# rhoposit/self-attention-tacotron

Hardware: AMD Instinct MI355X
Metric: teacher-forced mel frames/sec, LJSpeech batch=32, 1/2/4/8 MI355X (higher is better)
Workload: dtype fp32; 1 GPU; LJSpeech self-attention-tacotron.json teacher-forced training step (fwd + BPTT + Adam), configs[1]; global_batch=32, per_gpu_batch=32, chars=200, mel_frames=1000, num_mels=80, r=2, decoder_steps=500, parallelism=dp1, hip_graph=True, params=6227928

## Files before the change

self-attention-tacotron_amd/csrc/decoder_persistent.hip:

```cpp
#include "sat_common.h"
#include "persistent.h"

namespace sat {
namespace {

constexpr int kG = 8;
constexpr int kGW = 32;
constexpr int kPN = 32;
constexpr int kUBmax = 4;
constexpr int kU = 256, kM1 = 256, kM2 = 32, kD1 = 224, kD2 = 32, kF = 5, kKW = 10;
constexpr int kK0 = kM1 + kM2 + kU;
constexpr int kKP = 576;
constexpr int kPST = 8 + kM1 + kM2;
constexpr int kP4 = kPST / 4;
constexpr int kQ = kD1 + kD2;
constexpr int kUW = kU / kGW;
constexpr int kPadL = (kKW - 1) / 2;
constexpr int kPadR = kKW - 1 - kPadL;
constexpr int kEH = 16;
constexpr int kAH = 2;
static_assert(kK0 <= kKP && kKP == 9 * 64 && kU % kGW == 0 && kQ == 256 && kPST % 4 == 0 &&
              kD1 % 4 == 0, "layout");

struct DecAttnP {
// ... 641 lines not shown
  p.B = a->B; p.N = a->N; p.T = a->T; p.ntiles = ntiles; p.UB = ceil_div(a->B, kG);
  p.u = a->u; p.zc = a->zc; p.zh = a->zh;
  p.X0 = a->X0; p.W0r = a->W0r; p.Wq1 = a->Wq1; p.Wq2 = a->Wq2;
  p.K1 = a->K1; p.V1 = a->V1; p.K2 = a->K2; p.V2 = a->V2; p.lengths = a->lengths;
  p.v1 = a->v1; p.b1 = a->b1; p.convW = a->convW; p.convb = a->convb; p.locW = a->locW;
  p.v2 = a->v2; p.mask_c = a->mask_c; p.mask_h = a->mask_h;
  p.REC0 = a->REC0; p.C0 = a->C0; p.H0RAW = a->H0RAW; p.G0 = a->G0; p.Q = a->Q;
  p.S1 = a->S1; p.AL1 = a->AL1; p.S2 = a->S2; p.ST = a->ST; p.LOC = a->LOC;
  p.HX = a->E;
  p.EH = a->E + hx_floats(a->B);
  p.AH = p.EH + eh_floats(a->B, ntiles);
  p.XID = reinterpret_cast<unsigned*>(p.AH + ah_floats(a->B, ntiles));
  p.PART = a->PART; p.QP = a->QP; p.err = a->err;
  p.flags = xcd_local_env();
  p.prof = reinterpret_cast<long long*>(a->prof);
  p.ZH = a->ZH;
  hipStream_t s = as_stream(stream);
  const int64_t e_total = hx_floats(a->B) + eh_floats(a->B, ntiles) + ah_floats(a->B, ntiles) +
                        kXidWords;
  if (zero_ranges(s, a->E, e_total, a->PART, (int64_t)2 * a->B * ntiles * kPST, a->QP,
                  (int64_t)2 * a->B * kGW * kQ, a->err, 2) != hipSuccess) {
    set_error("sat_decoder_attention_fwd: memset failed");
    return SAT_ERR_HIP;
  }
  hipLaunchKernelGGL(dec_attn_fwd_kernel, dim3(kG * kGW), dim3(256), 0, s, p);
  SAT_LAUNCH_CHECK("sat_decoder_attention_fwd");
  return SAT_OK;
}

extern "C" int64_t sat_decoder_attention_scratch(int32_t B, int32_t N, int64_t* e_floats,
                                                 int64_t* part_floats, int64_t* qp_floats) {
  const int ntiles = ceil_div(N, kPN);
  if (e_floats) *e_floats = hx_floats(B) + eh_floats(B, ntiles) + ah_floats(B, ntiles) + kXidWords;
  if (part_floats) *part_floats = (int64_t)2 * B * ntiles * kPST;
  if (qp_floats) *qp_floats = (int64_t)2 * B * kGW * kQ;
  return kG * 64;
}
```

self-attention-tacotron_amd/csrc/decoder_persistent8.hip:

```cpp
#include "sat_common.h"
#include "persistent.h"

#ifndef SAT_FWD8_TRACE
#define SAT_FWD8_TRACE 0
#endif
#ifndef SAT_FWD8_NORM3
#define SAT_FWD8_NORM3 1
#endif
#ifndef SAT_FWD8_HSTORE7
#define SAT_FWD8_HSTORE7 1
#endif
#ifndef SAT_FWD8_ESCALE
#define SAT_FWD8_ESCALE 1
#endif
#ifndef SAT_FWD8_POLL1
#define SAT_FWD8_POLL1 1
#endif
#ifndef SAT_FWD8_HMERGE
#define SAT_FWD8_HMERGE 1
#endif

#ifndef SAT_FWD8_R1
#define SAT_FWD8_R1 1
#endif
#ifndef SAT_FWD8_R2
#define SAT_FWD8_R2 1
#endif
#ifndef SAT_FWD8_STW
#define SAT_FWD8_STW 1
#endif
#ifndef SAT_FWD8_R4
#define SAT_FWD8_R4 0
#endif
#ifndef SAT_FWD8_C2W
#define SAT_FWD8_C2W 0
#endif

namespace sat {
namespace {

constexpr int kW = 8;
constexpr int kGmax = 32;
constexpr int kTh = 512;
constexpr int kU = 256, kM1 = 256, kM2 = 32, kD1 = 224, kD2 = 32, kF = 5, kKW = 10;
constexpr int kC = kM1 + kM2;
constexpr int kK0 = kC + kU;
constexpr int kQ = kD1 + kD2;
constexpr int kUW = kU / kW;
constexpr int kPmax = 32;
constexpr int kPadL = (kKW - 1) / 2;
constexpr int kPadR = kKW - 1 - kPadL;
constexpr int kRA = kQ + kUW;
constexpr int kRB = 320;
constexpr int kRBctx = 8, kRBeh = kRBctx + kC, kRBet = kRBeh + kPadR, kRBal = kRBet + kPadL;
constexpr int kR4 = 2 + kC / 4;
constexpr float kTwoLog2e = 2.8853900817779268f;
static_assert(kRBal + 2 <= kRB && kK0 == 544 && kQ == 256 && kD1 % 16 == 0, "layout");

struct Fwd8P {
  int B, N, T, P, flags;
  float u, zc, zh;
  const float* X0; const float* W0r; const float* Wq1; const float* Wq2;
  const float* K1; const float* V1; const float* K2; const float* V2;
  const int64_t* lengths;
  const float* v1; const float* b1; const float* convW; const float* convb; const float* locW;
  const float* v2;
  const float* mask_c; const float* mask_h;
  float* REC0; float* C0; float* H0RAW; float* G0; float* Q;
  float* S1; float* AL1; float* S2; float* ST; float* LOC; float* ZH;
  float* RA;
  float* RB;
  unsigned* XID;
  int* err;
  long long* prof;
};

typedef float f2 __attribute__((ext_vector_type(2)));
typedef float f4v __attribute__((ext_vector_type(4)));

__device__ __forceinline__ bool any_lane(bool v) { return __builtin_amdgcn_ballot_w64(v) != 0; }
__device__ __forceinline__ float rdl(float v, int l) {
  return __int_as_float(__builtin_amdgcn_readlane(__float_as_int(v), l));
}
__device__ __forceinline__ float4 add4(float4 a, float4 b) {
  return make_float4(a.x + b.x, a.y + b.y, a.z + b.z, a.w + b.w);
}
__device__ __forceinline__ float sigm_fast(float x) {
  return __builtin_amdgcn_rcpf(1.f + __expf(-x));
}
__device__ __forceinline__ float fold32(float x) {
  const auto r = __builtin_amdgcn_permlane32_swap(__float_as_uint(x), __float_as_uint(x), false, false);
  return __uint_as_float(r[0]) + __uint_as_float(r[1]);
}
__device__ __forceinline__ float4 quad_gather(float x) {
  return make_float4(x, dpp_mov<0x101>(x), dpp_mov<0x102>(x), dpp_mov<0x103>(x));
}

__global__ void __launch_bounds__(kTh) dec_attn_fwd8_kernel(Fwd8P p) {
  __shared__ __attribute__((aligned(16))) float kc[kPmax][kQ];
  __shared__ __attribute__((aligned(16))) float v1s[kPmax][kM1];
  __shared__ __attribute__((aligned(16))) float v2s[kPmax][kM2];
  __shared__ __attribute__((aligned(16))) float wqs[kUW][kQ];
  __shared__ __attribute__((aligned(16))) float wc2[kM2][4 * kUW + 4];
  __shared__ __attribute__((aligned(16))) float cwl[kKW][kQ];
  __shared__ __attribute__((aligned(16))) float vcat[kQ];
  __shared__ float cw[kKW * kF + kF];
  __shared__ __attribute__((aligned(16))) float hbuf[kU];
  __shared__ __attribute__((aligned(16))) float cbuf[kC];
  __shared__ __attribute__((aligned(16))) float4 qst[kW][64];
  __shared__ __attribute__((aligned(16))) float4 recs[kW][kR4];
  __shared__ __attribute__((aligned(16))) float hst[kUW];
  __shared__ __attribute__((aligned(16))) float hraw[kUW];
  __shared__ float cown[kUW];
  __shared__ __attribute__((aligned(16))) float4 gown[kUW];
  __shared__ float gsum[8][64];
  __shared__ float halo[12];
  __shared__ float eown[kPmax], e2own[kPmax];
  __shared__ float alf[2][kPmax + 1];
  __shared__ float sp[kPmax + kKW];
  __shared__ __attribute__((aligned(16))) float wsc[8][2][kPmax];
  __shared__ long long tp[16];

  const int tid0 = threadIdx.x;
  const int g = blockIdx.x % kGmax, j = blockIdx.x / kGmax;
  const int B = p.B, N = p.N, T = p.T, P = p.P;
  if (g >= B) return;
  const int b = g;
  const int n0 = j * P, nt = max(0, min(P, N - n0));
  const bool has_left = j > 0, has_right = j + 1 < kW && n0 + P < N;
  const bool w7_stores = SAT_FWD8_HSTORE7 && 4 * 7 >= nt;
  const int64_t bN = (int64_t)b * N;
  const int len = (int)p.lengths[b];
  const float u = p.u;
  const auto rRA = rsrc(p.RA), rRB = rsrc(p.RB);

  f2 w0[8][8];
  {
    const int lane = tid0 & 63, wave = tid0 >> 6;
#pragma unroll
    for (int i = 0; i < 8; ++i) {
      const int r = i < 4 ? kC + 64 * i + lane : 64 * (i - 4) + lane;
      const float4* src = reinterpret_cast<const float4*>(p.W0r + (int64_t)r * (4 * kU) +
                                                          128 * j + 16 * wave);
#pragma unroll
      for (int q = 0; q < 4; ++q) {
        const float4 a = src[q];
        w0[i][2 * q] = f2{a.x, a.y};
        w0[i][2 * q + 1] = f2{a.z, a.w};
      }
    }
  }
  for (int i = tid0; i < kM2 * 32; i += kTh) {
    const int r = i >> 5, c4 = i & 31;
    *reinterpret_cast<float4*>(&wc2[r][4 * c4]) =
        reinterpret_cast<const float4*>(p.W0r + (int64_t)(kM1 + r) * (4 * kU) + 128 * j)[c4];
  }
  for (int i = tid0; i < kUW * kQ; i += kTh) {
    const int uu = i / kQ, c = i - uu * kQ, k = kUW * j + uu;
    wqs[uu][c] = c < kD1 ? p.Wq1[k * kD1 + c] : p.Wq2[k * kD2 + (c - kD1)];
  }
  for (int i = tid0; i < kPmax * kQ; i += kTh) {
    const int r = i / kQ, c = i - r * kQ;
    float lb = 0.f;
    if (c < kD1) {
#pragma unroll
      for (int f = 0; f < kF; ++f) lb = fmaf(p.convb[f], p.locW[f * kD1 + c], lb);
    }
    const float kv = r >= nt ? 0.f : c < kD1 ? p.K1[(bN + n0 + r) * kD1 + c] + p.b1[c] + lb
                                            : p.K2[(bN + n0 + r) * kD2 + (c - kD1)];
    kc[r][c] = SAT_FWD8_ESCALE ? kv * kTwoLog2e : kv;
  }
  for (int i = tid0; i < kKW * kQ; i += kTh) {
    const int k = i / kQ, c = i - k * kQ;
    float a = 0.f;
    if (c < kD1) {
#pragma unroll
      for (int f = 0; f < kF; ++f) a = fmaf(p.convW[k * kF + f], p.locW[f * kD1 + c], a);
    }
    cwl[k][c] = SAT_FWD8_ESCALE ? a * kTwoLog2e : a;
  }
  for (int i = tid0; i < kPmax * kM1 / 4; i += kTh) {
    const int r = i / (kM1 / 4), c4 = i - r * (kM1 / 4);
    reinterpret_cast<float4*>(&v1s[r][0])[c4] = r < nt
        ? reinterpret_cast<const float4*>(p.V1 + (bN + n0 + r) * kM1)[c4] : make_float4(0, 0, 0, 0);
  }
  for (int i = tid0; i < kPmax * kM2; i += kTh) {
    const int r = i / kM2, c = i - r * kM2;
    v2s[r][c] = r < nt ? p.V2[(bN + n0 + r) * kM2 + c] : 0.f;
  }
  for (int d = tid0; d < kQ; d += kTh) vcat[d] = d < kD1 ? p.v1[d] : p.v2[d - kD1];
  if (tid0 < kKW * kF) cw[tid0] = p.convW[tid0];
  if (tid0 < kF) cw[kKW * kF + tid0] = p.convb[tid0];
  if (tid0 < kU) hbuf[tid0] = 0.f;
  if (tid0 < 16) tp[tid0] = 0;
  gsum[tid0 >> 6][tid0 & 63] = 0.f;
  if (tid0 < nt + kKW - 1) {
    const int n = n0 - kPadL + tid0;
    sp[tid0] = (n >= 0 && n < N) ? p.S1[bN + n] : 0.f;
  }
  if (tid0 >= 64 && tid0 - 64 <= nt) {
    const int n = n0 - 1 + (tid0 - 64);
    alf[0][tid0 - 64] = tagf(n >= 0 ? p.AL1[bN + n] : 0.f, lsb_tag(0));
  }
  float c_own = 0.f, h_own = 0.f;
  const bool masked = p.mask_c != nullptr;
  auto load_ops = [&](int tt, int lane_, int wave_, float& xg_, float& mc_, float& mh_) {
    const int m = lane_ >> 2;
    const int64_t bu = ((int64_t)(tt < T ? tt : 0) * B + b) * kU + kUW * j + 4 * wave_ + (m >> 2);
    xg_ = p.X0[4 * bu + (m & 3)];
    const bool cl = (lane_ & 15) == 0 && masked;
    mc_ = cl ? p.mask_c[bu] : 1.f - p.zc;
    mh_ = cl ? p.mask_h[bu] : 1.f - p.zh;
  };
  float xgn, mcn, mhn;
  load_ops(0, tid0 & 63, tid0 >> 6, xgn, mcn, mhn);
  __syncthreads();

  const bool xl = (p.flags & 1) ? xcd_local_group(p.XID, g, kGmax, kW, p.err) : false;

#if SAT_FWD8_TRACE || SAT_SEGMENT_CLOCKS
  long long t0 = p.prof ? wall_clock64() : 0;
  auto tick = [&](int seg) {
    if (p.prof && tid0 == 0) {
      const long long t1 = wall_clock64();
      tp[seg] += t1 - t0;
      t0 = t1;
    }
  };
#else
  auto tick = [](int) {};
#endif
  bool gave_up = false;
  auto store_loc = [&](int tt, int lane_) {
    if (!p.LOC) return;
#pragma unroll
    for (int h = 0; h < 2; ++h) {
      const int o = lane_ + 64 * h;
      if (o < nt * kF) {
        const int i = o / kF, f = o - i * kF;
        float a = cw[kKW * kF + f];
#pragma unroll
        for (int k = 0; k < kKW; ++k) a = fmaf(sp[i + k], cw[k * kF + f], a);
        p.LOC[(((int64_t)tt * B + b) * N + n0) * kF + o] = a;
      }
    }
  };
  if ((tid0 >> 6) == 5) store_loc(0, tid0 & 63);
#if SAT_FWD8_TRACE
  long long* evt = (p.prof && blockIdx.x == 1) ? p.prof + 256 * 16 : nullptr;
  long long* gevt = (p.prof && g == 0) ? p.prof + 256 * 16 + 8 * 8 * 20 + j * 4 : nullptr;
#endif

  auto e_at = [&](int n) -> float {
    if (n < 0 || n >= len) return -INFINITY;
    if (n < n0) return halo[n - n0 + kPadL];
    if (n < n0 + nt) return eown[n - n0];
    return halo[kPadL + (n - n0 - nt)];
  };
  auto store_hist = [&](int tt, int lane_, float M1, float Z1, float A1, float M2, float Z2) {
    const int ss = tt - 1;
    if (lane_ >= kPadL && lane_ < nt + kPadL) {
      const float e = e_at(n0 - kPadL + lane_);
      p.S1[((int64_t)tt * B + b) * N + n0 + lane_ - kPadL] =
          e == -INFINITY ? 0.f : __expf(e - M1) * __builtin_amdgcn_rcpf(Z1);
    }
    if (lane_ < nt) {
      const float e2 = e2own[lane_];
      p.S2[((int64_t)ss * B + b) * N + n0 + lane_] =
          e2 == -INFINITY ? 0.f : __expf(e2 - M2) * __builtin_amdgcn_rcpf(Z2);
    }
    if (j == 0 && lane_ == 0) {
      float* stp = p.ST + ((int64_t)ss * B + b) * 4;
      stp[0] = M1; stp[1] = Z1; stp[2] = A1 / Z1; stp[3] = Z2;
    }
  };

  for (int t = 0; t <= T; ++t) {
    const int s = t - 1;
    float M1 = 0.f, Z1 = 1.f, A1 = 1.f, M2 = 0.f, Z2 = 1.f;
    int tid = tid0;
    asm volatile("" : "+v"(tid));
    const int lane = tid & 63;
    const int wave = __builtin_amdgcn_readfirstlane(tid >> 6);
    auto ev = [&](int k) {
#if SAT_FWD8_TRACE
      if (evt && t >= 100 && t < 108 && lane == 0) evt[((t - 100) * 8 + wave) * 16 + k] = wall_clock64();
      if (gevt && t >= 100 && t < 108 && tid == 0 && (k == 7 || k == 10 || k == 15 || k == 2)) {
        const int slot = k == 7 ? 0 : k == 10 ? 1 : k == 15 ? 2 : 3;
        const int ts = k == 2 ? t - 1 : t;
        if (ts >= 100) gevt[(ts - 100) * 32 + slot] = wall_clock64();
      }
#else
      (void)k;
#endif
    };
    ev(0);
    if (t > 0) {
      const int rb0 = ((s & 1) * B + b) * kW;
      const unsigned want = lsb_tag(s);
      const int rec = (rb0 + wave) * kRB;
      const bool two = lane < kM2 / 4 + 2;
      const int i2 = lane < kM2 / 4 ? (rec + kRBctx + kM1) / 4 + lane : rec / 4 + (lane - kM2 / 4);
      const int hq = lane - 16;
      const bool hl = wave == 0 && hq >= 0 && hq < 11;
      const bool hleft = hq < kPadL || hq >= kPadL + kPadR;
      const bool hsrc = hl && (hleft ? has_left : has_right);
      const int hw = (rb0 + (hleft ? j - 1 : j + 1)) * kRB +
                     (hq < kPadL ? kRBet + hq : hq < kPadL + kPadR ? kRBeh + hq - kPadL
                                                                   : kRBal + hq - kPadL - kPadR);
      float4 x1 = make_float4(0.f, 0.f, 0.f, 0.f), x2 = x1;
      float hv = 0.f;
      bool ok1 = false, ok2 = !two, ok3 = !hsrc;
#if SAT_FWD8_TRACE
      const long long tq0 = wall_clock64();
      asm volatile("s_waitcnt vmcnt(0)" ::: "memory");
      const long long tq1 = wall_clock64();
#endif
      bool retry = true;
      if (SAT_FWD8_POLL1) {
        x1 = ldc4(rRB, (rec + kRBctx) / 4 + lane);
        x2 = ldc4(rRB, i2);
        const float h0 = ldc(rRB, hsrc ? hw : 0);
        hv = hsrc ? h0 : 0.f;
        ok1 = tag_ok4(x1, want);
        ok2 = ok2 || tag_ok4(x2, want);
        ok3 = ok3 || tag_ok(hv, want);
        retry = any_lane(!(ok1 && ok2 && ok3)) && !gave_up;
      }
      if (retry) {
        for (unsigned spins = 0;; ++spins) {
          if (!ok1) x1 = ldc4(rRB, (rec + kRBctx) / 4 + lane);
          if (!ok2) x2 = ldc4(rRB, i2);
          if (!ok3) hv = ldc(rRB, hsrc ? hw : 0);
          ok1 = tag_ok4(x1, want);
          ok2 = ok2 || tag_ok4(x2, want);
          ok3 = ok3 || tag_ok(hv, want);
          if (!any_lane(!(ok1 && ok2 && ok3)) || gave_up) break;
          if (poll_give_up(spins, p.err)) { gave_up = true; break; }
          __builtin_amdgcn_s_sleep(1);
        }
      }
#if SAT_FWD8_TRACE
      {
        const long long tq2 = wall_clock64();
        if (evt && t >= 100 && t < 108 && lane == 0) {
          evt[8 * 8 * 16 + ((t - 100) * 8 + wave) * 4 + 0] = tq1 - tq0;
          evt[8 * 8 * 16 + ((t - 100) * 8 + wave) * 4 + 1] = tq2 - tq1;
        }
      }
#endif
      recs[wave][2 + lane] = x1;
      if (lane < kM2 / 4) recs[wave][2 + kM1 / 4 + lane] = x2;
      else if (two) recs[wave][lane - kM2 / 4] = x2;
      if (hl) halo[hq] = hv;
      tick(0);
    ev(1);
      lds_barrier();
      tick(1);
    ev(2);
      {
        const int jj = lane & 7;
        const float4 st = recs[jj][0];
        const float z2 = recs[jj][1].x;
        M1 = lanes8_max(st.x);
        M2 = lanes8_max(st.w);
        const float sc1 = __expf(st.x - M1), sc2 = __expf(st.w - M2);
        Z1 = lanes8_sum(st.y * sc1);
        A1 = lanes8_sum(st.z * sc1);
        Z2 = lanes8_sum(z2 * sc2);
        if (wave < (kC + 63) / 64) {
          if (tid < kC) {
            const bool first = wave < kM1 / 64;
            const float sc = first ? sc1 : sc2;
            const float* rf = reinterpret_cast<const float*>(&recs[0][2]) + tid;
            float a = 0.f;
#pragma unroll
            for (int k = 0; k < kW; ++k) a = fmaf(rf[k * kR4 * 4], rdl(sc, k), a);
            a *= __builtin_amdgcn_rcpf(first ? A1 : Z2);
            cbuf[tid] = a;
            if (tid / (kC / kW) == j) p.REC0[((int64_t)t * B + b) * kK0 + tid] = a;
          }
        } else {
          const unsigned bit = lsb_tag(t);
          if (wave == 5) {
            if (lane < nt + kKW - 1) {
              const float e = e_at(n0 - kPadL + lane);
              const float sv = e == -INFINITY ? 0.f : __expf(e - M1) * __builtin_amdgcn_rcpf(Z1);
              sp[lane] = sv;
              if (!SAT_FWD8_NORM3 && lane >= kPadL && lane < nt + kPadL)
                p.S1[((int64_t)t * B + b) * N + n0 + lane - kPadL] = sv;
            }
            if (t < T && 4 * 7 < nt) {
              asm volatile("s_waitcnt lgkmcnt(0)" ::: "memory");
              store_loc(t, lane);
            }
          } else if (wave == 6) {
            const float* ap = alf[(t - 1) & 1];
            if (lane <= nt) {
              const int k = lane, n = n0 - 1 + k;
              float av = 0.f;
              if (n >= 0) {
                const float a_n = k >= 1 ? ap[k] : halo[kPadL + kPadR + 1];
                const float a_m = k >= 2 ? ap[k - 1] : halo[kPadL + kPadR + k];
                const float e = e_at(n);
                const float pe = e == -INFINITY ? 0.f : __expf(e - M1);
                av = ((1.f - u) * a_n + u * a_m + 1e-7f) * pe * __builtin_amdgcn_rcpf(A1);
              }
              const float at = tagf(av, bit);
              alf[t & 1][k] = at;
              if (k >= 1 && !(SAT_FWD8_R4 && w7_stores && t < T))
                p.AL1[((int64_t)t * B + b) * N + n] = at;
            }
          }
          const bool defer = SAT_FWD8_R1 && w7_stores && t < T;
          if (SAT_FWD8_NORM3 ? (wave == 7 && !defer) : wave == 6) {
            if (SAT_FWD8_NORM3) {
              store_hist(t, lane, M1, Z1, A1, M2, Z2);
            } else {
              if (lane < nt) {
                const float e2 = e2own[lane];
                p.S2[((int64_t)s * B + b) * N + n0 + lane] =
                    e2 == -INFINITY ? 0.f : __expf(e2 - M2) * __builtin_amdgcn_rcpf(Z2);
              }
              if (j == 0 && lane == 0) {
                float* stp = p.ST + ((int64_t)s * B + b) * 4;
                stp[0] = M1; stp[1] = Z1; stp[2] = A1 / Z1; stp[3] = Z2;
              }
            }
          }
        }
      }
    }
    tick(2);
    ev(3);
    lds_barrier();
    tick(3);
    ev(4);

    if (t < T) {
      f2 acc[8];
#pragma unroll
      for (int q = 0; q < 8; ++q) acc[q] = f2{0.f, 0.f};
      if (t > 0) {
#if SAT_FWD8_HMERGE
#pragma unroll
        for (int i = 0; i < 4; ++i) {
          const float xv = hbuf[64 * i + lane];
          const f2 xx = {xv, xv};
#pragma unroll
          for (int q = 0; q < 8; ++q) acc[q] = __builtin_elementwise_fma(xx, w0[i][q], acc[q]);
        }
#endif
#pragma unroll
        for (int i = 4; i < 8; ++i) {
          const float xv = cbuf[64 * (i - 4) + lane];
          const f2 xx = {xv, xv};
#pragma unroll
          for (int q = 0; q < 8; ++q) acc[q] = __builtin_elementwise_fma(xx, w0[i][q], acc[q]);
        }
        const int r2 = lane & 31, hsel = lane >> 5;
        const float xv = cbuf[kM1 + r2];
        const f2 xx = {xv, xv};
        const float4 wa = *reinterpret_cast<const float4*>(&wc2[r2][16 * wave + 8 * hsel]);
        const float4 wb = *reinterpret_cast<const float4*>(&wc2[r2][16 * wave + 8 * hsel + 4]);
        const f2 c0 = __builtin_elementwise_fma(xx, f2{wa.x, wa.y}, f2{0.f, 0.f});
        const f2 c1 = __builtin_elementwise_fma(xx, f2{wa.z, wa.w}, f2{0.f, 0.f});
        const f2 c2 = __builtin_elementwise_fma(xx, f2{wb.x, wb.y}, f2{0.f, 0.f});
        const f2 c3 = __builtin_elementwise_fma(xx, f2{wb.z, wb.w}, f2{0.f, 0.f});
        if (hsel == 0) { acc[0] += c0; acc[1] += c1; acc[2] += c2; acc[3] += c3; }
        else { acc[4] += c0; acc[5] += c1; acc[6] += c2; acc[7] += c3; }
      }
      float v[16];
#pragma unroll
      for (int q = 0; q < 8; ++q) { v[2 * q] = acc[q].x; v[2 * q + 1] = acc[q].y; }
      transpose_reduce16(v, lane);
      const int gate = (lane >> 2) & 3;
#if SAT_FWD8_HMERGE
      const float pre = v[0] + xgn;
#else
      const float pre = v[0] + gsum[wave][lane] + xgn;
#endif
      const float sg = sigm_fast(gate == 1 ? 2.f * pre : pre + (gate == 2 ? 1.0f : 0.f));
      const float act = gate == 1 ? fmaf(2.f, sg, -1.f) : sg;
      const float gj = dpp_mov<0x104>(act);
      const float gf = dpp_mov<0x108>(act);
      const float go = dpp_mov<0x10C>(act);
      const bool cell = (lane & 15) == 0;
      const int cq = lane >> 4, cunit = kUW * j + 4 * wave + cq;
      const float mc = mcn, mh = mhn;
      const unsigned bit = lsb_tag(t);
      if (cell) {
        const float gi = act;
        const float cn = gf * c_own + gi * gj;
        const float hn = go * fmaf(2.f, sigm_fast(2.f * cn), -1.f);
// ... 17 lines not shown
      tick(4);
    ev(5);
      lds_barrier();
      tick(5);
    ev(6);
      {
        const int col = 32 * wave + (lane & 31), u0 = 16 * (lane >> 5);
        float a = 0.f;
#pragma unroll
        for (int k4 = 0; k4 < 4; ++k4) {
          const float4 h4 = *reinterpret_cast<const float4*>(&hraw[u0 + 4 * k4]);
          a = fmaf(h4.x, wqs[u0 + 4 * k4][col], a);
          a = fmaf(h4.y, wqs[u0 + 4 * k4 + 1][col], a);
          a = fmaf(h4.z, wqs[u0 + 4 * k4 + 2][col], a);
          a = fmaf(h4.w, wqs[u0 + 4 * k4 + 3][col], a);
        }
        const float4 q4 = quad_gather(fold32(a));
        const int ra = (((t & 1) * B + b) * kW + j) * kRA;
        if (lane < 32 && (lane & 3) == 0) stc4x(xl, rRA, ra / 4 + 8 * wave + (lane >> 2), tagf4(q4, bit));
        if (wave == 1 && lane < kUW / 4)
          stc4x(xl, rRA, (ra + kQ) / 4 + lane, *reinterpret_cast<const float4*>(&hst[4 * lane]));
      }
      tick(6);
    ev(7);
    }

    if (t == T) break;
    tick(7);
    ev(8);

    float4 Lr[4];
    if (SAT_FWD8_R1 && SAT_FWD8_NORM3 && w7_stores && wave == 7 && t > 0)
      store_hist(t, lane, M1, Z1, A1, M2, Z2);
    if (SAT_FWD8_R4 && w7_stores && wave == 7 && t > 0 && lane >= 1 && lane <= nt &&
        n0 - 1 + lane >= 0)
      p.AL1[((int64_t)t * B + b) * N + n0 - 1 + lane] = alf[t & 1][lane];
    if (4 * wave < nt) {
      const int c = lane;
#pragma unroll
      for (int i = 0; i < 4; ++i) Lr[i] = *reinterpret_cast<const float4*>(&kc[4 * wave + i][4 * c]);
#pragma unroll
      for (int k = 0; k < kKW; ++k) {
        const float4 wk = *reinterpret_cast<const float4*>(&cwl[k][4 * c]);
#pragma unroll
        for (int i = 0; i < 4; ++i) {
          const float sv = sp[4 * wave + i + k];
          Lr[i].x = fmaf(sv, wk.x, Lr[i].x); Lr[i].y = fmaf(sv, wk.y, Lr[i].y);
          Lr[i].z = fmaf(sv, wk.z, Lr[i].z); Lr[i].w = fmaf(sv, wk.w, Lr[i].w);
        }
      }
    }
    tick(8);
    ev(9);

    {
      const unsigned want = lsb_tag(t);
      const int ra = (((t & 1) * B + b) * kW + wave) * kRA;
      const bool two = lane < kUW / 4;
      float4 x1 = make_float4(0.f, 0.f, 0.f, 0.f), x2 = x1;
      bool ok1 = false, ok2 = !two;
#if SAT_FWD8_TRACE
      const long long tq0 = wall_clock64();
      asm volatile("s_waitcnt vmcnt(0)" ::: "memory");
      const long long tq1 = wall_clock64();
#endif
      bool retry = true;
      if (SAT_FWD8_POLL1) {
        x1 = ldc4(rRA, ra / 4 + lane);
        x2 = ldc4(rRA, (ra + kQ) / 4 + (two ? lane : 0));
// ... 67 lines not shown
        const bool valid = r < nt && n0 + r < len;
        const float ev = valid ? tagf(e[0], bit) : -INFINITY;
        if (m < 4) eown[r] = ev; else e2own[r] = ev;
      }
    } else {
      const int r = 4 * wave + (lane & 3);
      if (lane < 4) eown[r] = -INFINITY; else if (lane < 8) e2own[r] = -INFINITY;
      if (wave == 0 && (lane >> 3) == j) {
        float4 q = qst[0][lane];
#pragma unroll
        for (int k = 1; k < kW; ++k) q = add4(q, qst[k][lane]);
        reinterpret_cast<float4*>(p.Q + ((int64_t)t * B + b) * kQ)[lane] = q;
      }
      if (wave == 7) {
        store_loc(t, lane);
        if (w7_stores && lane < kUW) {
          const int cunit = kUW * j + lane;
          const int64_t tbu = ((int64_t)t * B + b) * kU + cunit;
          p.C0[((int64_t)(t + 1) * B + b) * kU + cunit] = cown[lane];
          p.REC0[((int64_t)(t + 1) * B + b) * kK0 + kC + cunit] = hst[lane];
          p.H0RAW[tbu] = hraw[lane];
          reinterpret_cast<float4*>(p.G0)[tbu] = gown[lane];
        }
      }
    }
    tick(11);
    ev(12);
    lds_barrier();
    tick(12);
    ev(13);
    {
      const unsigned bit = lsb_tag(t);
      const float* al = alf[t & 1];
      if (SAT_FWD8_R2 && wave == 7 && lane < kPadR + kPadL + 2) {
        const int rb = (((t & 1) * B + b) * kW + j) * kRB;
        const int q = lane;
        float v;
        if (q < kPadR) v = q < nt ? eown[q] : -INFINITY;
        else if (q < kPadR + kPadL) { const int i = nt - kPadL + (q - kPadR); v = i >= 0 ? eown[i] : -INFINITY; }
        else { const int k = nt - 1 + (q - kPadR - kPadL); v = k >= 0 ? al[k] : 0.f; }
        stcx(xl, rRB, rb + kRBeh + q, tagf(v == -INFINITY ? 0.f : v, bit));
      }
      const float e1v = lane < kPmax ? eown[lane] : -INFINITY;
      const float e2v = lane < kPmax ? e2own[lane] : -INFINITY;
      const float m1 = tagf(fmaxf(wave_max_dpp(e1v), -3.402823466e38f), bit);
      const float m2 = tagf(fmaxf(wave_max_dpp(e2v), -3.402823466e38f), bit);
      const float pe = e1v == -INFINITY ? 0.f : __expf(e1v - m1);
      const float pe2 = e2v == -INFINITY ? 0.f : __expf(e2v - m2);
      const float w = lane < nt ? ((1.f - u) * al[lane + 1] + u * al[lane] + 1e-7f) * pe : 0.f;
      if (lane < kPmax) { wsc[wave][0][lane] = w; wsc[wave][1][lane] = lane < nt ? pe2 : 0.f; }
      if (wave == SAT_FWD8_STW) {
        const float z1 = tagf(wave_sum_dpp(pe), bit), a1 = tagf(wave_sum_dpp(w), bit);
        const float z2 = tagf(wave_sum_dpp(pe2), bit);
        if (lane == 0) {
          const int rb = (((t & 1) * B + b) * kW + j) * kRB;
          stc4x(xl, rRB, rb / 4, make_float4(m1, z1, a1, m2));
          stc4x(xl, rRB, rb / 4 + 1, tagf4(make_float4(z2, 0.f, 0.f, 0.f), bit));
        }
      }
      asm volatile("s_waitcnt lgkmcnt(0)" ::: "memory");
    }
    tick(13);
    ev(14);
    {
      const unsigned bit = lsb_tag(t);
      const int rb = (((t & 1) * B + b) * kW + j) * kRB;
      const int col = lane & 31, r0 = 16 * (lane >> 5);
      const float* ws = &wsc[wave][0][r0];
      float c = 0.f;
#pragma unroll
      for (int k4 = 0; k4 < 4; ++k4) {
        const float4 w4 = *reinterpret_cast<const float4*>(ws + 4 * k4);
        c = fmaf(w4.x, v1s[r0 + 4 * k4][32 * wave + col], c);
        c = fmaf(w4.y, v1s[r0 + 4 * k4 + 1][32 * wave + col], c);
        c = fmaf(w4.z, v1s[r0 + 4 * k4 + 2][32 * wave + col], c);
        c = fmaf(w4.w, v1s[r0 + 4 * k4 + 3][32 * wave + col], c);
      }
      const float4 c4 = quad_gather(fold32(c));
      if (lane < 32 && (lane & 3) == 0)
        stc4x(xl, rRB, (rb + kRBctx) / 4 + 8 * wave + (lane >> 2), tagf4(c4, bit));
      if (wave == SAT_FWD8_C2W) {
        const float* ws2 = &wsc[SAT_FWD8_C2W][1][r0];
        float c2 = 0.f;
#pragma unroll
        for (int k = 0; k < 16; ++k) c2 = fmaf(ws2[k], v2s[r0 + k][col], c2);
        const float4 q4 = quad_gather(fold32(c2));
        if (lane < 32 && (lane & 3) == 0)
          stc4x(xl, rRB, (rb + kRBctx + kM1) / 4 + (lane >> 2), tagf4(q4, bit));
      } else if (!SAT_FWD8_R2 && wave == 1 && lane < kPadR + kPadL + 2) {
        const int q = lane;
        float v;
        if (q < kPadR) v = q < nt ? eown[q] : -INFINITY;
        else if (q < kPadR + kPadL) { const int i = nt - kPadL + (q - kPadR); v = i >= 0 ? eown[i] : -INFINITY; }
        else { const int k = nt - 1 + (q - kPadR - kPadL); v = k >= 0 ? alf[t & 1][k] : 0.f; }
        stcx(xl, rRB, rb + kRBeh + q, tagf(v == -INFINITY ? 0.f : v, bit));
      }
    }
    tick(14);
    ev(15);
    if (!SAT_FWD8_HMERGE && t + 1 < T) {
      f2 acc[8];
#pragma unroll
      for (int q = 0; q < 8; ++q) acc[q] = f2{0.f, 0.f};
#pragma unroll
      for (int i = 0; i < 4; ++i) {
        const float xv = hbuf[64 * i + lane];
        const f2 xx = {xv, xv};
#pragma unroll
        for (int q = 0; q < 8; ++q) acc[q] = __builtin_elementwise_fma(xx, w0[i][q], acc[q]);
      }
      float v[16];
#pragma unroll
      for (int q = 0; q < 8; ++q) { v[2 * q] = acc[q].x; v[2 * q + 1] = acc[q].y; }
      transpose_reduce16(v, lane);
      gsum[wave][lane] = v[0];
    }
    tick(15);
  }
#if SAT_FWD8_TRACE || SAT_SEGMENT_CLOCKS
  if (p.prof && tid0 == 0)
    for (int i = 0; i < 16; ++i) p.prof[blockIdx.x * 16 + i] = tp[i];
#endif
}

}

bool dec_attn_fwd8_eligible(const SatDecAttnFwd* a) {
  return a->U == kU && a->M1 == kM1 && a->M2 == kM2 && a->D1 == kD1 && a->D2 == kD2 &&
         a->F == kF && a->KW == kKW && a->B >= 1 && a->B <= kGmax && a->N >= 1 &&
         a->N <= kW * kPmax;
}

int dec_attn_fwd8_launch(const SatDecAttnFwd* a, hipStream_t s) {
  int dev = 0, cus = 0, per_cu = 0;
  if (hipGetDevice(&dev) != hipSuccess ||
      hipDeviceGetAttribute(&cus, hipDeviceAttributeMultiprocessorCount, dev) != hipSuccess ||
      hipOccupancyMaxActiveBlocksPerMultiprocessor(&per_cu, dec_attn_fwd8_kernel, kTh, 0) != hipSuccess) {
    set_error("sat_decoder_attention_fwd: device query failed");
    return SAT_ERR_HIP;
  }
  SAT_CHECK_ARG((int64_t)cus * per_cu >= kGmax * kW,
                "sat_decoder_attention_fwd: fewer than 256 co-resident workgroups on this device");
  Fwd8P p;
  p.B = a->B; p.N = a->N; p.T = a->T;
  p.P = std::max(kPadR, ceil_div(a->N, kW));
  p.u = a->u; p.zc = a->zc; p.zh = a->zh;
  p.X0 = a->X0; p.W0r = a->W0r; p.Wq1 = a->Wq1; p.Wq2 = a->Wq2;
  p.K1 = a->K1; p.V1 = a->V1; p.K2 = a->K2; p.V2 = a->V2; p.lengths = a->lengths;
  p.v1 = a->v1; p.b1 = a->b1; p.convW = a->convW; p.convb = a->convb; p.locW = a->locW;
  p.v2 = a->v2; p.mask_c = a->mask_c; p.mask_h = a->mask_h;
  p.REC0 = a->REC0; p.C0 = a->C0; p.H0RAW = a->H0RAW; p.G0 = a->G0; p.Q = a->Q;
  p.S1 = a->S1; p.AL1 = a->AL1; p.S2 = a->S2; p.ST = a->ST; p.LOC = a->LOC; p.ZH = a->ZH;
  const int64_t ra = (int64_t)2 * a->B * kW * kRA, rb = (int64_t)2 * a->B * kW * kRB;
  p.RA = a->QP;
  p.RB = a->QP + ra;
  p.XID = reinterpret_cast<unsigned*>(a->QP + ra + rb);
  p.err = a->err;
  p.flags = xcd_local_env();
  p.prof = reinterpret_cast<long long*>(a->prof);
  if (zero_ranges(s, a->QP, ra + rb + kGmax * kW, a->err, 2) != hipSuccess) {
    set_error("sat_decoder_attention_fwd: scratch clear failed");
    return SAT_ERR_HIP;
  }
  hipLaunchKernelGGL(dec_attn_fwd8_kernel, dim3(kGmax * kW), dim3(kTh), 0, s, p);
  SAT_LAUNCH_CHECK("sat_decoder_attention_fwd");
  return SAT_OK;
}

}
```

self-attention-tacotron_amd/csrc/persistent.h:

```cpp
#pragma once
#include "sat_common.h"
#include <cstdlib>

namespace sat {
namespace {

typedef unsigned v4u __attribute__((ext_vector_type(4)));

__device__ __forceinline__ __amdgpu_buffer_rsrc_t rsrc(const void* base) {
  return __builtin_amdgcn_make_buffer_rsrc(const_cast<void*>(base), 0, 0x7fffffff, 0x00020000);
}
__device__ __forceinline__ float ldc(__amdgpu_buffer_rsrc_t r, int idx) {
  return __uint_as_float(__builtin_amdgcn_raw_buffer_load_b32(r, idx * 4, 0, 16));
}
__device__ __forceinline__ float4 ldc4(__amdgpu_buffer_rsrc_t r, int idx4) {
  const v4u v = __builtin_amdgcn_raw_buffer_load_b128(r, idx4 * 16, 0, 16);
  return make_float4(__uint_as_float(v[0]), __uint_as_float(v[1]), __uint_as_float(v[2]),
                     __uint_as_float(v[3]));
}
__device__ __forceinline__ void stc(__amdgpu_buffer_rsrc_t r, int idx, float v) {
  __builtin_amdgcn_raw_buffer_store_b32(__float_as_uint(v), r, idx * 4, 0, 16);
}
__device__ __forceinline__ void stc4(__amdgpu_buffer_rsrc_t r, int idx4, float4 v) {
  const v4u w = {__float_as_uint(v.x), __float_as_uint(v.y), __float_as_uint(v.z),
// ... 165 lines not shown
  tr_dpp<2, 1>(v, lane);
  v[0] += dpp_mov<0xB1>(v[0]);
}
__device__ __forceinline__ void transpose_reduce8(float* v, int lane) {
#pragma unroll
  for (int i = 0; i < 4; ++i) v[i] = fsum_swap32(v[i], v[i + 4]);
#pragma unroll
  for (int i = 0; i < 2; ++i) v[i] = fsum_swap16(v[i], v[i + 2]);
  tr_dpp<8, 1>(v, lane);
  {
    const float up = dpp_mov<0x104>(v[0]), dn = dpp_mov<0x114>(v[0]);
    v[0] += (lane & 4) ? dn : up;
  }
  v[0] += dpp_mov<0x4E>(v[0]);
  v[0] += dpp_mov<0xB1>(v[0]);
}
__device__ __forceinline__ void transpose_reduce16(float* v, int lane) {
#pragma unroll
  for (int i = 0; i < 8; ++i) v[i] = fsum_swap32(v[i], v[i + 8]);
#pragma unroll
  for (int i = 0; i < 4; ++i) v[i] = fsum_swap16(v[i], v[i + 4]);
  tr_dpp<8, 2>(v, lane);
  tr_dpp<4, 1>(v, lane);
  v[0] += dpp_mov<0xB1>(v[0]);
  v[0] += dpp_mov<0x4E>(v[0]);
}

}
}

namespace sat {
bool dec_attn_fwd8_eligible(const SatDecAttnFwd* a);
int dec_attn_fwd8_launch(const SatDecAttnFwd* a, hipStream_t s);
bool dec_attn_bwd8_eligible(const SatDecAttnBwd* a);
int dec_attn_bwd8_launch(const SatDecAttnBwd* a, hipStream_t s);
}
```

Baseline: 2.429 million frames/s.

## Precompute V1·W0r so the persistent decoder exchanges attention weights instead of contexts

```diff
diff --git a/self-attention-tacotron_amd/csrc/decoder_persistent.hip b/self-attention-tacotron_amd/csrc/decoder_persistent.hip
--- a/self-attention-tacotron_amd/csrc/decoder_persistent.hip
+++ b/self-attention-tacotron_amd/csrc/decoder_persistent.hip
@@ -697,7 +697,8 @@
                                                  int64_t* part_floats, int64_t* qp_floats) {
   const int ntiles = ceil_div(N, kPN);
   if (e_floats) *e_floats = hx_floats(B) + eh_floats(B, ntiles) + ah_floats(B, ntiles) + kXidWords;
-  if (part_floats) *part_floats = (int64_t)2 * B * ntiles * kPST;
+  if (part_floats)
+    *part_floats = std::max((int64_t)2 * B * ntiles * kPST, dec_attn_fwd8_part_floats(B, N));
   if (qp_floats) *qp_floats = (int64_t)2 * B * kGW * kQ;
   return kG * 64;
 }
diff --git a/self-attention-tacotron_amd/csrc/decoder_persistent8.hip b/self-attention-tacotron_amd/csrc/decoder_persistent8.hip
--- a/self-attention-tacotron_amd/csrc/decoder_persistent8.hip
+++ b/self-attention-tacotron_amd/csrc/decoder_persistent8.hip
@@ -22,18 +22,6 @@
 
 #ifndef SAT_FWD8_R1
 #define SAT_FWD8_R1 1
-#endif
-#ifndef SAT_FWD8_R2
-#define SAT_FWD8_R2 1
-#endif
-#ifndef SAT_FWD8_STW
-#define SAT_FWD8_STW 1
-#endif
-#ifndef SAT_FWD8_R4
-#define SAT_FWD8_R4 0
-#endif
-#ifndef SAT_FWD8_C2W
-#define SAT_FWD8_C2W 0
 #endif
 
 namespace sat {
@@ -51,17 +39,18 @@
 constexpr int kPadL = (kKW - 1) / 2;
 constexpr int kPadR = kKW - 1 - kPadL;
 constexpr int kRA = kQ + kUW;
-constexpr int kRB = 320;
-constexpr int kRBctx = 8, kRBeh = kRBctx + kC, kRBet = kRBeh + kPadR, kRBal = kRBet + kPadL;
-constexpr int kR4 = 2 + kC / 4;
+constexpr int kRB = 96;
+constexpr int kRBw = 8, kRBc2 = kRBw + kPmax, kRBeh = kRBc2 + kM2, kRBet = kRBeh + kPadR,
+              kRBal = kRBet + kPadL;
+constexpr int kR4 = kRBeh / 4;
 constexpr float kTwoLog2e = 2.8853900817779268f;
-static_assert(kRBal + 2 <= kRB && kK0 == 544 && kQ == 256 && kD1 % 16 == 0, "layout");
+static_assert(kRBal + 2 <= kRB && kRB % 4 == 0 && kR4 == 18 && kR4 <= 64 && kK0 == 544 && kQ == 256 && kD1 % 16 == 0, "layout");
 
 struct Fwd8P {
   int B, N, T, P, flags;
   float u, zc, zh;
   const float* X0; const float* W0r; const float* Wq1; const float* Wq2;
-  const float* K1; const float* V1; const float* K2; const float* V2;
+  const float* K1; const float* VW1; const float* K2; const float* V2;
   const int64_t* lengths;
   const float* v1; const float* b1; const float* convW; const float* convb; const float* locW;
   const float* v2;
@@ -98,7 +87,6 @@
 
 __global__ void __launch_bounds__(kTh) dec_attn_fwd8_kernel(Fwd8P p) {
   __shared__ __attribute__((aligned(16))) float kc[kPmax][kQ];
-  __shared__ __attribute__((aligned(16))) float v1s[kPmax][kM1];
   __shared__ __attribute__((aligned(16))) float v2s[kPmax][kM2];
   __shared__ __attribute__((aligned(16))) float wqs[kUW][kQ];
   __shared__ __attribute__((aligned(16))) float wc2[kM2][4 * kUW + 4];
@@ -106,7 +94,8 @@
   __shared__ __attribute__((aligned(16))) float vcat[kQ];
   __shared__ float cw[kKW * kF + kF];
   __shared__ __attribute__((aligned(16))) float hbuf[kU];
-  __shared__ __attribute__((aligned(16))) float cbuf[kC];
+  __shared__ __attribute__((aligned(16))) float abuf[kW * kPmax];
+  __shared__ __attribute__((aligned(16))) float c2buf[kM2];
   __shared__ __attribute__((aligned(16))) float4 qst[kW][64];
   __shared__ __attribute__((aligned(16))) float4 recs[kW][kR4];
   __shared__ __attribute__((aligned(16))) float hst[kUW];
@@ -118,7 +107,7 @@
   __shared__ float eown[kPmax], e2own[kPmax];
   __shared__ float alf[2][kPmax + 1];
   __shared__ float sp[kPmax + kKW];
-  __shared__ __attribute__((aligned(16))) float wsc[8][2][kPmax];
+  __shared__ __attribute__((aligned(16))) float w2s[kPmax];
   __shared__ long long tp[16];
 
   const int tid0 = threadIdx.x;
@@ -139,12 +128,14 @@
     const int lane = tid0 & 63, wave = tid0 >> 6;
 #pragma unroll
     for (int i = 0; i < 8; ++i) {
-      const int r = i < 4 ? kC + 64 * i + lane : 64 * (i - 4) + lane;
-      const float4* src = reinterpret_cast<const float4*>(p.W0r + (int64_t)r * (4 * kU) +
-                                                          128 * j + 16 * wave);
+      const int n = 64 * (i - 4) + lane;
+      const bool live = i < 4 || n < N;
+      const float* row = i < 4 ? p.W0r + (int64_t)(kC + 64 * i + lane) * (4 * kU)
+                               : p.VW1 + (bN + (live ? n : 0)) * (4 * kU);
+      const float4* src = reinterpret_cast<const float4*>(row + 128 * j + 16 * wave);
 #pragma unroll
       for (int q = 0; q < 4; ++q) {
-        const float4 a = src[q];
+        const float4 a = live ? src[q] : make_float4(0.f, 0.f, 0.f, 0.f);
         w0[i][2 * q] = f2{a.x, a.y};
         w0[i][2 * q + 1] = f2{a.z, a.w};
       }
@@ -179,11 +170,6 @@
     }
     cwl[k][c] = SAT_FWD8_ESCALE ? a * kTwoLog2e : a;
   }
-  for (int i = tid0; i < kPmax * kM1 / 4; i += kTh) {
-    const int r = i / (kM1 / 4), c4 = i - r * (kM1 / 4);
-    reinterpret_cast<float4*>(&v1s[r][0])[c4] = r < nt
-        ? reinterpret_cast<const float4*>(p.V1 + (bN + n0 + r) * kM1)[c4] : make_float4(0, 0, 0, 0);
-  }
   for (int i = tid0; i < kPmax * kM2; i += kTh) {
     const int r = i / kM2, c = i - r * kM2;
     v2s[r][c] = r < nt ? p.V2[(bN + n0 + r) * kM2 + c] : 0.f;
@@ -192,6 +178,7 @@
   if (tid0 < kKW * kF) cw[tid0] = p.convW[tid0];
   if (tid0 < kF) cw[kKW * kF + tid0] = p.convb[tid0];
   if (tid0 < kU) hbuf[tid0] = 0.f;
+  if (tid0 < kW * kPmax) abuf[tid0] = 0.f;
   if (tid0 < 16) tp[tid0] = 0;
   gsum[tid0 >> 6][tid0 & 63] = 0.f;
   if (tid0 < nt + kKW - 1) {
@@ -234,7 +221,7 @@
   auto store_loc = [&](int tt, int lane_) {
     if (!p.LOC) return;
 #pragma unroll
-    for (int h = 0; h < 2; ++h) {
+    for (int h = 0; h < (kPmax * kF + 63) / 64; ++h) {
       const int o = lane_ + 64 * h;
       if (o < nt * kF) {
         const int i = o / kF, f = o - i * kF;
@@ -299,8 +286,8 @@
       const int rb0 = ((s & 1) * B + b) * kW;
       const unsigned want = lsb_tag(s);
       const int rec = (rb0 + wave) * kRB;
-      const bool two = lane < kM2 / 4 + 2;
-      const int i2 = lane < kM2 / 4 ? (rec + kRBctx + kM1) / 4 + lane : rec / 4 + (lane - kM2 / 4);
+      const bool one = lane < kR4;
+      const int i1 = rec / 4 + (one ? lane : 0);
       const int hq = lane - 16;
       const bool hl = wave == 0 && hq >= 0 && hq < 11;
       const bool hleft = hq < kPadL || hq >= kPadL + kPadR;
@@ -308,9 +295,9 @@
       const int hw = (rb0 + (hleft ? j - 1 : j + 1)) * kRB +
                      (hq < kPadL ? kRBet + hq : hq < kPadL + kPadR ? kRBeh + hq - kPadL
                                                                    : kRBal + hq - kPadL - kPadR);
-      float4 x1 = make_float4(0.f, 0.f, 0.f, 0.f), x2 = x1;
+      float4 x1 = make_float4(0.f, 0.f, 0.f, 0.f);
       float hv = 0.f;
-      bool ok1 = false, ok2 = !two, ok3 = !hsrc;
+      bool ok1 = !one, ok3 = !hsrc;
 #if SAT_FWD8_TRACE
       const long long tq0 = wall_clock64();
       asm volatile("s_waitcnt vmcnt(0)" ::: "memory");
@@ -318,24 +305,20 @@
 #endif
       bool retry = true;
       if (SAT_FWD8_POLL1) {
-        x1 = ldc4(rRB, (rec + kRBctx) / 4 + lane);
-        x2 = ldc4(rRB, i2);
+        x1 = ldc4(rRB, i1);
         const float h0 = ldc(rRB, hsrc ? hw : 0);
         hv = hsrc ? h0 : 0.f;
-        ok1 = tag_ok4(x1, want);
-        ok2 = ok2 || tag_ok4(x2, want);
+        ok1 = ok1 || tag_ok4(x1, want);
         ok3 = ok3 || tag_ok(hv, want);
-        retry = any_lane(!(ok1 && ok2 && ok3)) && !gave_up;
+        retry = any_lane(!(ok1 && ok3)) && !gave_up;
       }
       if (retry) {
         for (unsigned spins = 0;; ++spins) {
-          if (!ok1) x1 = ldc4(rRB, (rec + kRBctx) / 4 + lane);
-          if (!ok2) x2 = ldc4(rRB, i2);
+          if (!ok1) x1 = ldc4(rRB, i1);
           if (!ok3) hv = ldc(rRB, hsrc ? hw : 0);
-          ok1 = tag_ok4(x1, want);
-          ok2 = ok2 || tag_ok4(x2, want);
+          ok1 = ok1 || tag_ok4(x1, want);
           ok3 = ok3 || tag_ok(hv, want);
-          if (!any_lane(!(ok1 && ok2 && ok3)) || gave_up) break;
+          if (!any_lane(!(ok1 && ok3)) || gave_up) break;
           if (poll_give_up(spins, p.err)) { gave_up = true; break; }
           __builtin_amdgcn_s_sleep(1);
         }
@@ -349,9 +332,7 @@
         }
       }
 #endif
-      recs[wave][2 + lane] = x1;
-      if (lane < kM2 / 4) recs[wave][2 + kM1 / 4 + lane] = x2;
-      else if (two) recs[wave][lane - kM2 / 4] = x2;
+      if (one) recs[wave][lane] = x1;
       if (hl) halo[hq] = hv;
       tick(0);
     ev(1);
@@ -368,17 +349,20 @@
         Z1 = lanes8_sum(st.y * sc1);
         A1 = lanes8_sum(st.z * sc1);
         Z2 = lanes8_sum(z2 * sc2);
-        if (wave < (kC + 63) / 64) {
-          if (tid < kC) {
-            const bool first = wave < kM1 / 64;
-            const float sc = first ? sc1 : sc2;
-            const float* rf = reinterpret_cast<const float*>(&recs[0][2]) + tid;
+        if (wave < kW * kPmax / 64) {
+          const int k = 2 * wave + (lane >> 5), i = lane & 31;
+          const float sk = lane < 32 ? rdl(sc1, 2 * wave) : rdl(sc1, 2 * wave + 1);
+          const float wv = reinterpret_cast<const float*>(&recs[k][0])[kRBw + i];
+          if (i < P && k * P + i < N) abuf[k * P + i] = wv * sk * __builtin_amdgcn_rcpf(A1);
+        } else if (wave == kW * kPmax / 64) {
+          if (lane < kM2) {
+            const float* rf = reinterpret_cast<const float*>(&recs[0][0]) + kRBc2 + lane;
             float a = 0.f;
 #pragma unroll
-            for (int k = 0; k < kW; ++k) a = fmaf(rf[k * kR4 * 4], rdl(sc, k), a);
-            a *= __builtin_amdgcn_rcpf(first ? A1 : Z2);
-            cbuf[tid] = a;
-            if (tid / (kC / kW) == j) p.REC0[((int64_t)t * B + b) * kK0 + tid] = a;
+            for (int k = 0; k < kW; ++k) a = fmaf(rf[k * kR4 * 4], rdl(sc2, k), a);
+            a *= __builtin_amdgcn_rcpf(Z2);
+            c2buf[lane] = a;
+            if (lane / (kM2 / kW) == j) p.REC0[((int64_t)t * B + b) * kK0 + kM1 + lane] = a;
           }
         } else {
           const unsigned bit = lsb_tag(t);
@@ -408,7 +392,7 @@
               }
               const float at = tagf(av, bit);
               alf[t & 1][k] = at;
-              if (k >= 1 && !(SAT_FWD8_R4 && w7_stores && t < T))
+              if (k >= 1)
                 p.AL1[((int64_t)t * B + b) * N + n] = at;
             }
           }
@@ -453,13 +437,13 @@
 #endif
 #pragma unroll
         for (int i = 4; i < 8; ++i) {
-          const float xv = cbuf[64 * (i - 4) + lane];
+          const float xv = abuf[64 * (i - 4) + lane];
           const f2 xx = {xv, xv};
 #pragma unroll
           for (int q = 0; q < 8; ++q) acc[q] = __builtin_elementwise_fma(xx, w0[i][q], acc[q]);
         }
         const int r2 = lane & 31, hsel = lane >> 5;
-        const float xv = cbuf[kM1 + r2];
+        const float xv = c2buf[r2];
         const f2 xx = {xv, xv};
         const float4 wa = *reinterpret_cast<const float4*>(&wc2[r2][16 * wave + 8 * hsel]);
         const float4 wb = *reinterpret_cast<const float4*>(&wc2[r2][16 * wave + 8 * hsel + 4]);
@@ -543,9 +527,6 @@
     float4 Lr[4];
     if (SAT_FWD8_R1 && SAT_FWD8_NORM3 && w7_stores && wave == 7 && t > 0)
       store_hist(t, lane, M1, Z1, A1, M2, Z2);
-    if (SAT_FWD8_R4 && w7_stores && wave == 7 && t > 0 && lane >= 1 && lane <= nt &&
-        n0 - 1 + lane >= 0)
-      p.AL1[((int64_t)t * B + b) * N + n0 - 1 + lane] = alf[t & 1][lane];
     if (4 * wave < nt) {
       const int c = lane;
 #pragma unroll
@@ -679,8 +660,8 @@
     {
       const unsigned bit = lsb_tag(t);
       const float* al = alf[t & 1];
-      if (SAT_FWD8_R2 && wave == 7 && lane < kPadR + kPadL + 2) {
-        const int rb = (((t & 1) * B + b) * kW + j) * kRB;
+      const int rb = (((t & 1) * B + b) * kW + j) * kRB;
+      if (wave == 7 && lane < kPadR + kPadL + 2) {
         const int q = lane;
         float v;
         if (q < kPadR) v = q < nt ? eown[q] : -INFINITY;
@@ -688,60 +669,43 @@
         else { const int k = nt - 1 + (q - kPadR - kPadL); v = k >= 0 ? al[k] : 0.f; }
         stcx(xl, rRB, rb + kRBeh + q, tagf(v == -INFINITY ? 0.f : v, bit));
       }
-      const float e1v = lane < kPmax ? eown[lane] : -INFINITY;
-      const float e2v = lane < kPmax ? e2own[lane] : -INFINITY;
-      const float m1 = tagf(fmaxf(wave_max_dpp(e1v), -3.402823466e38f), bit);
-      const float m2 = tagf(fmaxf(wave_max_dpp(e2v), -3.402823466e38f), bit);
-      const float pe = e1v == -INFINITY ? 0.f : __expf(e1v - m1);
-      const float pe2 = e2v == -INFINITY ? 0.f : __expf(e2v - m2);
-      const float w = lane < nt ? ((1.f - u) * al[lane + 1] + u * al[lane] + 1e-7f) * pe : 0.f;
-      if (lane < kPmax) { wsc[wave][0][lane] = w; wsc[wave][1][lane] = lane < nt ? pe2 : 0.f; }
-      if (wave == SAT_FWD8_STW) {
-        const float z1 = tagf(wave_sum_dpp(pe), bit), a1 = tagf(wave_sum_dpp(w), bit);
-        const float z2 = tagf(wave_sum_dpp(pe2), bit);
-        if (lane == 0) {
-          const int rb = (((t & 1) * B + b) * kW + j) * kRB;
-          stc4x(xl, rRB, rb / 4, make_float4(m1, z1, a1, m2));
-          stc4x(xl, rRB, rb / 4 + 1, tagf4(make_float4(z2, 0.f, 0.f, 0.f), bit));
-        }
-      }
-      asm volatile("s_waitcnt lgkmcnt(0)" ::: "memory");
+      if (wave <= 1) {
+        const float e2v = lane < kPmax ? e2own[lane] : -INFINITY;
+        const float m2 = tagf(fmaxf(wave_max_dpp(e2v), -3.402823466e38f), bit);
+        const float pe2 = e2v == -INFINITY ? 0.f : __expf(e2v - m2);
+        if (wave == 1) {
+          const float e1v = lane < kPmax ? eown[lane] : -INFINITY;
+          const float m1 = tagf(fmaxf(wave_max_dpp(e1v), -3.402823466e38f), bit);
+          const float pe = e1v == -INFINITY ? 0.f : __expf(e1v - m1);
+          const float w = lane < nt ? tagf(((1.f - u) * al[lane + 1] + u * al[lane] + 1e-7f) * pe, bit) : 0.f;
+          const float z1 = tagf(wave_sum_dpp(pe), bit), a1 = tagf(wave_sum_dpp(w), bit);
+          const float z2 = tagf(wave_sum_dpp(pe2), bit);
+          const float4 w4 = quad_gather(w);
+          if (lane < kPmax && (lane & 3) == 0)
+            stc4x(xl, rRB, (rb + kRBw) / 4 + (lane >> 2), tagf4(w4, bit));
+          if (lane == 0) {
+            stc4x(xl, rRB, rb / 4, make_float4(m1, z1, a1, m2));
+            stc4x(xl, rRB, rb / 4 + 1, tagf4(make_float4(z2, 0.f, 0.f, 0.f), bit));
+          }
+        } else {
+          if (lane < kPmax) w2s[lane] = lane < nt ? pe2 : 0.f;
+          asm volatile("s_waitcnt lgkmcnt(0)" ::: "memory");
+        }
+      }
     }
     tick(13);
     ev(14);
-    {
+    if (wave == 0) {
       const unsigned bit = lsb_tag(t);
       const int rb = (((t & 1) * B + b) * kW + j) * kRB;
       const int col = lane & 31, r0 = 16 * (lane >> 5);
-      const float* ws = &wsc[wave][0][r0];
-      float c = 0.f;
-#pragma unroll
-      for (int k4 = 0; k4 < 4; ++k4) {
-        const float4 w4 = *reinterpret_cast<const float4*>(ws + 4 * k4);
-        c = fmaf(w4.x, v1s[r0 + 4 * k4][32 * wave + col], c);
-        c = fmaf(w4.y, v1s[r0 + 4 * k4 + 1][32 * wave + col], c);
-        c = fmaf(w4.z, v1s[r0 + 4 * k4 + 2][32 * wave + col], c);
-        c = fmaf(w4.w, v1s[r0 + 4 * k4 + 3][32 * wave + col], c);
-      }
-      const float4 c4 = quad_gather(fold32(c));
+      const float* ws2 = &w2s[r0];
+      float c2 = 0.f;
+#pragma unroll
+      for (int k = 0; k < 16; ++k) c2 = fmaf(ws2[k], v2s[r0 + k][col], c2);
+      const float4 q4 = quad_gather(fold32(c2));
       if (lane < 32 && (lane & 3) == 0)
-        stc4x(xl, rRB, (rb + kRBctx) / 4 + 8 * wave + (lane >> 2), tagf4(c4, bit));
-      if (wave == SAT_FWD8_C2W) {
-        const float* ws2 = &wsc[SAT_FWD8_C2W][1][r0];
-        float c2 = 0.f;
-#pragma unroll
-        for (int k = 0; k < 16; ++k) c2 = fmaf(ws2[k], v2s[r0 + k][col], c2);
-        const float4 q4 = quad_gather(fold32(c2));
-        if (lane < 32 && (lane & 3) == 0)
-          stc4x(xl, rRB, (rb + kRBctx + kM1) / 4 + (lane >> 2), tagf4(q4, bit));
-      } else if (!SAT_FWD8_R2 && wave == 1 && lane < kPadR + kPadL + 2) {
-        const int q = lane;
-        float v;
-        if (q < kPadR) v = q < nt ? eown[q] : -INFINITY;
-        else if (q < kPadR + kPadL) { const int i = nt - kPadL + (q - kPadR); v = i >= 0 ? eown[i] : -INFINITY; }
-        else { const int k = nt - 1 + (q - kPadR - kPadL); v = k >= 0 ? alf[t & 1][k] : 0.f; }
-        stcx(xl, rRB, rb + kRBeh + q, tagf(v == -INFINITY ? 0.f : v, bit));
-      }
+        stc4x(xl, rRB, (rb + kRBc2) / 4 + (lane >> 2), tagf4(q4, bit));
     }
     tick(14);
     ev(15);
@@ -778,7 +742,14 @@
          a->N <= kW * kPmax;
 }
 
+int64_t dec_attn_fwd8_part_floats(int B, int N) {
+  return (B >= 1 && B <= kGmax && N >= 1 && N <= kW * kPmax) ? (int64_t)B * N * 4 * kU : 0;
+}
+
 int dec_attn_fwd8_launch(const SatDecAttnFwd* a, hipStream_t s) {
+  SAT_CHECK_ARG(a->PART != nullptr && aligned16(a->PART),
+                "sat_decoder_attention_fwd: PART (the V1 . W0r product's scratch) must be "
+                "non-null and 16-byte aligned");
   int dev = 0, cus = 0, per_cu = 0;
   if (hipGetDevice(&dev) != hipSuccess ||
       hipDeviceGetAttribute(&cus, hipDeviceAttributeMultiprocessorCount, dev) != hipSuccess ||
@@ -793,7 +764,7 @@
   p.P = std::max(kPadR, ceil_div(a->N, kW));
   p.u = a->u; p.zc = a->zc; p.zh = a->zh;
   p.X0 = a->X0; p.W0r = a->W0r; p.Wq1 = a->Wq1; p.Wq2 = a->Wq2;
-  p.K1 = a->K1; p.V1 = a->V1; p.K2 = a->K2; p.V2 = a->V2; p.lengths = a->lengths;
+  p.K1 = a->K1; p.VW1 = a->PART; p.K2 = a->K2; p.V2 = a->V2; p.lengths = a->lengths;
   p.v1 = a->v1; p.b1 = a->b1; p.convW = a->convW; p.convb = a->convb; p.locW = a->locW;
   p.v2 = a->v2; p.mask_c = a->mask_c; p.mask_h = a->mask_h;
   p.REC0 = a->REC0; p.C0 = a->C0; p.H0RAW = a->H0RAW; p.G0 = a->G0; p.Q = a->Q;
@@ -809,9 +780,24 @@
     set_error("sat_decoder_attention_fwd: scratch clear failed");
     return SAT_ERR_HIP;
   }
+  SatGemmDesc d;
+  std::memset(&d, 0, sizeof(d));
+  d.M = a->B * a->N; d.N = 4 * kU; d.K = kM1; d.batch = 1; d.batch2 = 1;
+  d.A = a->V1; d.a_sm = kM1; d.a_sk = 1;
+  d.B = a->W0r; d.b_sk = 4 * kU; d.b_sn = 1;
+  d.C = a->PART; d.c_sm = 4 * kU;
+  d.alpha = 1.f; d.beta = 0.f;
+  int rc = sat_gemm(&d, s);
+  if (rc != SAT_OK) return rc;
   hipLaunchKernelGGL(dec_attn_fwd8_kernel, dim3(kGmax * kW), dim3(kTh), 0, s, p);
   SAT_LAUNCH_CHECK("sat_decoder_attention_fwd");
-  return SAT_OK;
-}
-
-}
+  std::memset(&d, 0, sizeof(d));
+  d.M = a->T; d.N = kM1; d.K = a->N; d.batch = a->B; d.batch2 = 1;
+  d.A = a->AL1 + (int64_t)a->B * a->N; d.a_sm = (int64_t)a->B * a->N; d.a_sk = 1; d.a_sbatch = a->N;
+  d.B = a->V1; d.b_sk = kM1; d.b_sn = 1; d.b_sbatch = (int64_t)a->N * kM1;
+  d.C = a->REC0 + (int64_t)a->B * kK0; d.c_sm = (int64_t)a->B * kK0; d.c_sbatch = kK0;
+  d.alpha = 1.f; d.beta = 0.f;
+  return sat_gemm(&d, s);
+}
+
+}
diff --git a/self-attention-tacotron_amd/csrc/persistent.h b/self-attention-tacotron_amd/csrc/persistent.h
--- a/self-attention-tacotron_amd/csrc/persistent.h
+++ b/self-attention-tacotron_amd/csrc/persistent.h
@@ -221,6 +221,7 @@
 namespace sat {
 bool dec_attn_fwd8_eligible(const SatDecAttnFwd* a);
 int dec_attn_fwd8_launch(const SatDecAttnFwd* a, hipStream_t s);
+int64_t dec_attn_fwd8_part_floats(int B, int N);
 bool dec_attn_bwd8_eligible(const SatDecAttnBwd* a);
 int dec_attn_bwd8_launch(const SatDecAttnBwd* a, hipStream_t s);
 }
```

After: 2.442 million frames/s (median of 6 runs). No clear change (+0.6%).
